# ErrorTzy/unpaper-gpu

Hardware: AMD Instinct MI355X
Metric: pages/sec + Mpixel/s, 1000-page GRAY8 A4@300dpi batch, 1/2/4/8 GPU (higher is better)
Workload: dtype u8; 1 GPU; 1000 synthetic GRAY8 A4@300dpi pages (2480x3508) per GPU, default pipeline, inputs and outputs resident in HBM; pages_per_gpu=1000, sheets_per_batch=64, streams=16, hw_queues=24, parallelism=one runner thread per device, pages sharded, no collective

## Files before the change

unpaper-gpu_amd/csrc/kernels_deskew.hip:

```cpp
#include <climits>
#include <mutex>
#include <vector>
#include <cmath>

#include "filters.h"
#include "libm_glibc.h"

namespace uph {

constexpr int kDepth = 128;
constexpr int kSliceRows = 128;
constexpr int kBandCapMax = 384;

__device__ __forceinline__ int iwave_prefix_excl(int v, int* total) {
  const int lane = threadIdx.x & 63;
  int pre = v;
  for (int o = 1; o < 64; o <<= 1) {
    int t = __shfl_up(pre, o, 64);
    if (lane >= o) pre += t;
  }
  *total = __shfl(pre, 63, 64);
  return pre - v;
}

// ... 112 lines not shown
    R.nseg[t] = 0;
    R.flag[t] = 1;
    if (act) R.list[atomicAdd(R.nlist, 1)] = t;
    return;
  }
  const LineSetup L = line_setup(masks[s], g, g.edge_shift[e][0], 0, table->slope[a]);
  const int scan = L.scan;
  int4* sg = R.segs + (int64_t)t * kLineSegs;
  int ns = 0, last = 0;
  bool over = false;
  float X = L.X;
  const float st = L.stepX;
  int i = 0;
  while (scan > 0) {
    if (ns >= kLineSegs) {
      over = true;
      break;
    }
    const float sign = X > 0.0f ? 1.0f : -1.0f;
    const double T = (double)fabsf(X), sig = (double)st * (double)sign;
    int64_t nn = 0;
    double du = 0.0;
    if (X != 0.0f) {
      int E;
      frexpf(fabsf(X), &E);
      if (E < -100) {
        over = true;
        break;
      }
      const double lo = ldexp(1.0, E - 1), hi = ldexp(1.0, E), u = ldexp(1.0, E - 24);
      const double q = ldexp(sig, 24 - E);
      const double fqd = floor(q);
      const int64_t fq = (int64_t)fqd;
      const bool tie = q - fqd == 0.5;
      if (!tie || !(((int64_t)ldexp(T, 24 - E)) & 1)) {
        const int64_t dq = tie ? (fq & 1 ? fq + 1 : fq) : (int64_t)floor(q + 0.5);
        const int64_t H = (int64_t)ldexp(hi - T, 24 - E), G = (int64_t)ldexp(T - lo, 24 - E);
        const int64_t rem = scan - 1 - i;
        auto div24 = [](int64_t c, int64_t d) -> int64_t {
          return d > c ? 0 : (int64_t)((uint32_t)c / (uint32_t)d);
        };
        if (dq > 0) {
          const int64_t c = H - fq - 1;
          nn = c >= 0 ? div24(c, dq) + 1 : 0;
        } else if (dq < 0) {
          const int64_t c = G + fq;
          nn = c >= 0 ? div24(c, -dq) + 1 : 0;
        } else {
          nn = (q >= 0.0 || G >= 1) ? rem : 0;
        }
        if (nn > rem) nn = rem;
        du = (double)dq * u;
      }
    }
    const float Ts = sign * (float)T, ds = sign * (float)du;
    sg[ns++] = make_int4(i, (int32_t)nn, __float_as_int(Ts), __float_as_int(ds));
    i += (int)nn;
    if (i >= scan - 1) {
      last = (int)fmaf((float)nn, ds, Ts);
      break;
    }
    X = sign * (float)(T + (double)nn * du) + st;
    i++;
  }
  const int first = scan > 0 ? (int)L.X : 0;
  R.ends[2 * t] = first;
  R.ends[2 * t + 1] = over ? first : last;
  const int se = t / na, lo = over ? first : imin(first, last), hi = over ? first : imax(first, last);
  atomicMin(&slo[se - se_base], lo);
  atomicMax(&shi[se - se_base], hi);
  R.nseg[t] = over ? 0 : ns;
  R.flag[t] = over;
  if (over) R.list[atomicAdd(R.nlist, 1)] = t;
  }();
  __syncthreads();
  const int tl = imin(nlines, (int)((blockIdx.x + 1) * blockDim.x)) - 1;
  const int ng = tl >= 0 ? tl / na - se_base + 1 : 0;
  if ((int)threadIdx.x < ng && slo[threadIdx.x] <= shi[threadIdx.x]) {
    atomicMin(&R.blo[se_base + threadIdx.x], slo[threadIdx.x]);
    atomicMax(&R.bhi[se_base + threadIdx.x], shi[threadIdx.x]);
  }
}

__device__ __forceinline__ bool band_range(const RotScratch& R, int tbase, int na, int sxh,
                                           int band_cap, int32_t* bx0, int32_t* bw) {
  const int se = tbase / na;
  int32_t lo = R.blo[se], hi = R.bhi[se];
  if (sxh > 0) hi += kDepth - 1;
  else lo -= kDepth - 1;
  *bx0 = lo;
  *bw = hi - lo + 1;
  return *bw <= band_cap && lo <= hi;
}

constexpr int kBandThreads = 512;
__global__ void __launch_bounds__(kBandThreads, 4)
    k_rot_band_g(PlaneRef img, RotGeom g, const RotTable* table, const Rect* masks,
                 const int32_t* mask_active, int count, int max_scan, RotScratch R, int fmt,
                 int band_cap) {
  const int sl = blockIdx.x, e = blockIdx.y, s = blockIdx.z;
  const int na = table->nangles;
  const int sxh = g.edge_shift[e][0];
  if (g.edge_shift[e][1] != 0 || (mask_active && !mask_active[s])) return;
  const Rect mask = masks[s];
  const LineSetup LS = line_setup(mask, g, sxh, 0, 0.0f);
  const int i0 = sl * kSliceRows, i1 = imin(LS.scan, i0 + kSliceRows);
  if (i0 >= i1) return;
  const int tbase = (s * g.nedges + e) * na;
  int32_t bx0, bw;
  if (!band_range(R, tbase, na, sxh, band_cap, &bx0, &bw)) return;
  extern __shared__ __attribute__((aligned(16))) uint16_t pre[];
  uint8_t* raw = reinterpret_cast<uint8_t*>(pre) + kSliceRows * bw;
  const Rect nm = normalize(mask);
  const int32_t xlo = imax(nm.x0, 0), xhi = imin(nm.x1, g.W - 1);
  const int32_t ylo = imax(nm.y0, 0), yhi = imin(nm.y1, g.H - 1);
  const int32_t ystart = (int32_t)LS.Y;
  const uint8_t* base = plane_ptr(img, s);
  const int rows = i1 - i0;
  {
    const int lane = threadIdx.x & 63, w = threadIdx.x >> 6;
    constexpr int kPer = kBandCapMax / 64;
    for (int r = w; r < rows; r += kBandThreads / 64) {
      const int32_t y = ystart + i0 + r;
      const bool rok = (y >= ylo) & (y <= yhi);
      const uint8_t* row = base + (int64_t)(rok ? y : ylo) * img.P.pitch;
      uint8_t v[kPer];
#pragma unroll
      for (int k = 0; k < kPer; k++) {
        const int c = lane + 64 * k;
        const int32_t x = bx0 + c;
        const bool ok = rok & (c < bw) & (x >= xlo) & (x <= xhi);
        const int32_t xo = ok ? x : xlo;
        uint32_t d;
        if (fmt == F_GRAY8) d = row[xo];
        else if (fmt == F_Y400A) d = row[2 * xo];
        else d = dark_of(load_px_row<F_RGB24>(row, xo));
        v[k] = (uint8_t)((255 - d) & -(int)ok);
      }
#pragma unroll
      for (int k = 0; k < kPer; k++) {
        const int c = lane + 64 * k;
        if (c < bw) raw[r * bw + c] = v[k];
      }
    }
  }
  __syncthreads();
  const int c = threadIdx.x;
  uint32_t acc = 0;
  for (int k0 = 0; k0 < kSliceRows; k0 += 32) {
    uint32_t colv[8];
    if (c < bw) {
#pragma unroll
      for (int k = 0; k < 8; k++) {
        uint32_t wv = 0;
#pragma unroll
        for (int j = 0; j < 4; j++) {
          const int r = k0 + 4 * k + j;
          wv |= (r < rows ? (uint32_t)raw[r * bw + c] : 0u) << (8 * j);
        }
        colv[k] = wv;
      }
    }
    __syncthreads();
    if (c < bw) {
#pragma unroll
      for (int k = 0; k < 8; k++) {
#pragma unroll
        for (int j = 0; j < 4; j++) {
          const int r = k0 + 4 * k + j;
          acc += (colv[k] >> (8 * j)) & 0xFFu;
          if (r < rows) pre[r * bw + c] = (uint16_t)acc;
        }
      }
    }
  }
  __syncthreads();
  const int lane = threadIdx.x & 63, w = threadIdx.x >> 6;
  constexpr int nw = kBandThreads / 64;
  const int32_t o0 = sxh * lane - bx0, o1 = sxh * (lane + 64) - bx0;
  const int ns = rot_slices(max_scan);
  for (int a = w; a < na; a += nw) {
    const int t = __builtin_amdgcn_readfirstlane(tbase + a);
    int32_t cA = 0, cB = 0;
    {
      const int nsg = __builtin_amdgcn_readfirstlane(R.nseg[t]);
      const int4 mine = lane < nsg ? R.segs[(int64_t)t * kLineSegs + lane] : make_int4(INT_MAX, 0, 0, 0);
      const int iA = i0 + lane, iB = i0 + 64 + lane;
      int q0 = 0;
      while (q0 + 1 < nsg && __builtin_amdgcn_readlane(mine.x, q0 + 1) <= i0) q0++;
      const int nxt = q0 + 1 < nsg ? __builtin_amdgcn_readlane(mine.x, q0 + 1) : INT_MAX;
      if (nxt >= i1) {
        const int b = __builtin_amdgcn_readlane(mine.x, q0);
        const float T = __int_as_float(__builtin_amdgcn_readlane(mine.z, q0));
        const float d = __int_as_float(__builtin_amdgcn_readlane(mine.w, q0));
        if (lane < rows) cA = (int)fmaf((float)(iA - b), d, T);
        if (lane + 64 < rows) cB = (int)fmaf((float)(iB - b), d, T);
      } else {
        int qA = q0, qB = q0;
        for (int q = q0 + 1; q < nsg; q++) {
          const int s0 = __builtin_amdgcn_readlane(mine.x, q);
          if (s0 >= i1) break;
          qA = iA >= s0 ? q : qA;
          qB = iB >= s0 ? q : qB;
        }
        const int bA = __shfl(mine.x, qA, 64), bB = __shfl(mine.x, qB, 64);
        const float TA = __int_as_float(__shfl(mine.z, qA, 64)), dA = __int_as_float(__shfl(mine.w, qA, 64));
        const float TB = __int_as_float(__shfl(mine.z, qB, 64)), dB = __int_as_float(__shfl(mine.w, qB, 64));
        if (lane < rows) cA = (int)fmaf((float)(iA - bA), dA, TA);
        if (lane + 64 < rows) cB = (int)fmaf((float)(iB - bB), dB, TB);
      }
    }
    const int32_t upA = __shfl_up(cA, 1, 64), upB = __shfl_up(cB, 1, 64);
    const int32_t lastA = __builtin_amdgcn_readlane(cA, 63);
    const bool stA = lane < rows && (lane == 0 || upA != cA);
    const bool stB = lane + 64 < rows && (lane == 0 ? lastA != cB : upB != cB);
    unsigned long long MA = __ballot(stA), MB = __ballot(stB);
    int acc0 = 0, acc1 = 0;
    int rs = 0;
    int32_t x = __builtin_amdgcn_readlane(cA, 0);
    MA &= MA - 1;
    for (;;) {
      int re;
      int32_t nx = 0;
      if (MA) {
        re = __ffsll((long long)MA) - 1;
        nx = __builtin_amdgcn_readlane(cA, re);
        MA &= MA - 1;
      } else if (MB) {
        const int b = __ffsll((long long)MB) - 1;
        re = 64 + b;
        nx = __builtin_amdgcn_readlane(cB, b);
        MB &= MB - 1;
      } else {
        re = rows;
      }
      const uint16_t* pe = pre + (re - 1) * bw + x;
      acc0 += pe[o0];
      acc1 += pe[o1];
      if (rs > 0) {
        const uint16_t* ps = pre + (rs - 1) * bw + x;
        acc0 -= ps[o0];
        acc1 -= ps[o1];
      }
      if (re >= rows) break;
      rs = re;
      x = nx;
    }
    uint16_t* P = R.part + ((int64_t)t * ns + sl) * kDepth;
    P[lane] = (uint16_t)acc0;
    P[lane + 64] = (uint16_t)acc1;
  }
}

__global__ void __launch_bounds__(256) k_rot_final(RotGeom g, const RotTable* table,
                                                   const Rect* masks, const int32_t* mask_active,
                                                   int mask_index, int32_t* peaks, int count,
                                                   int max_scan, RotScratch R, int band_cap) {
  const int na = table->nangles;
  const int nlines = count * g.nedges * na;
  const int t = blockIdx.x * 4 + (threadIdx.x >> 6);
  const int lane = threadIdx.x & 63;
  if (t >= nlines) return;
  const int a = t % na, e = (t / na) % g.nedges, s = t / (na * g.nedges);
  int32_t* out = peaks + (((int64_t)s * g.max_masks + mask_index) * 4 + e) * na + a;
  if (mask_active && !mask_active[s]) {
    if (lane == 0) *out = 0;
    return;
  }
  if (R.flag[t]) return;
  const int sxh = g.edge_shift[e][0];
  const LineSetup LS = line_setup(masks[s], g, sxh, 0, table->slope[a]);
  int32_t bx0, bw;
  if (LS.scan <= 0) {
    if (lane == 0) *out = 0;
    return;
  }
  if (!band_range(R, (s * g.nedges + e) * na, na, sxh, band_cap, &bx0, &bw)) {
    if (lane == 0) {
      R.flag[t] = 1;
      R.list[atomicAdd(R.nlist, 1)] = t;
    }
    return;
  }
  const int ns = rot_slices(max_scan), nsl = (LS.scan + kSliceRows - 1) / kSliceRows;
  int B[2] = {0, 0};
#pragma unroll 4
  for (int q = 0; q < nsl; q++) {
    const uint32_t v = reinterpret_cast<const uint32_t*>(R.part + ((int64_t)t * ns + q) * kDepth)[lane];
    B[0] += (int)(v & 0xFFFFu);
    B[1] += (int)(v >> 16);
  }
  const int maxAbs = (int)(255 * g.scan_size * g.scan_depth);
  const int pre1 = B[0] + B[1];
  int tot;
  const int ex = iwave_prefix_excl(pre1, &tot);
  int kfail = 2;
  for (int k = 1; k >= 0; k--) {
    const int before = ex + (k ? B[0] : 0);
    if (!(before < maxAbs && 2 * lane + k < LS.maxDepth)) kfail = k;
  }
  const unsigned long long F = __ballot(kfail < 2);
  if (!F) {
    const int up1 = __shfl_up(B[1], 1, 64);
    const int prev0 = lane == 0 ? 0 : up1;
    int md = max(B[0] - prev0, B[1] - B[0]);
    for (int o = 32; o > 0; o >>= 1) md = max(md, __shfl_xor(md, o, 64));
    const int last = __shfl(B[1], 63, 64);
    if (lane == 0) {
      R.state[4 * t] = tot;
      R.state[4 * t + 1] = last;
      R.state[4 * t + 2] = md > 0 ? md : 0;
      R.state[4 * t + 3] = 1;
      R.flag[t] = 1;
      R.list[atomicAdd(R.nlist, 1)] = t;
    }
    return;
  }
  const int fl = __ffsll((long long)F) - 1;
  const int stop = 2 * fl + __shfl(kfail, fl, 64);
  const int up = __shfl_up(B[1], 1, 64);
  int prev = lane == 0 ? 0 : up;
  int md = INT_MIN;
  for (int k = 0; k < 2; k++) {
    if (2 * lane + k < stop) md = max(md, B[k] - prev);
    prev = B[k];
  }
  for (int o = 32; o > 0; o >>= 1) md = max(md, __shfl_xor(md, o, 64));
  const int maxDiff = md > 0 ? md : 0;
  if (lane == 0) *out = stop < LS.maxDepth ? maxDiff : 0;
// ... 52 lines not shown
    const int32_t ystart = (int32_t)LS.Y;
    for (int i = threadIdx.x; i < scan; i += blockDim.x) {
      px[i] = seg_col(segs_s, nsg, i);
      py[i] = ystart + i;
    }
  } else if (threadIdx.x == 0) {
    float X = LS.X, Y = LS.Y;
    for (int i = 0; i < scan; i++) {
      px[i] = (int)X;
      py[i] = (int)Y;
      X += LS.stepX;
      Y += LS.stepY;
    }
  }
  if (threadIdx.x == 0) {
    done_flag = 0;
    result = 0;
  }
  __syncthreads();
  const int lane = threadIdx.x & 63, w = threadIdx.x >> 6;
  const uint8_t* base = plane_ptr(img, s);
  const Rect nm = normalize(mask);
  int carry_acc = 0, last = 0, maxDiff = 0;
  int dstart = 0;
  if (resume) {
    carry_acc = R.state[4 * t];
    last = R.state[4 * t + 1];
    maxDiff = R.state[4 * t + 2];
    dstart = kDepth;
  }
  for (int d0 = dstart; d0 < maxDepth; d0 += 64) {
    const int dep = d0 + lane;
    int acc = 0;
#pragma unroll 8
    for (int i = w; i < scan; i += kWaves) {
      const int32_t x = px[i] + sxh * dep, y = py[i] + syv * dep;
      const bool ok = (x >= nm.x0) & (x <= nm.x1) & (y >= nm.y0) & (y <= nm.y1) & (x >= 0) &
                      (y >= 0) & (x < g.W) & (y < g.H);
      const Px p = load_px_row<FMT>(base + (int64_t)(ok ? y : 0) * img.P.pitch, ok ? x : 0);
      acc += (255 - (int)dark_of(p)) & -(int)ok;
    }
    part[w][lane] = acc;
    __syncthreads();
    if (w == 0) {
      int B = 0;
#pragma unroll
      for (int k = 0; k < kWaves; k++) B += part[k][lane];
      int tot;
      const int before = carry_acc + iwave_prefix_excl(B, &tot);
      const bool exec = before < maxAbs && dep < maxDepth;
      const unsigned long long X_ = __ballot(!exec);
      const int stop = X_ ? __ffsll((long long)X_) - 1 : 64;
      const int up = __shfl_up(B, 1, 64);
      const int prevB = lane == 0 ? last : up;
      const int diff = B - prevB;
      int md = lane < stop ? diff : INT_MIN;
      for (int o = 32; o > 0; o >>= 1) md = max(md, __shfl_xor(md, o, 64));
      if (md > maxDiff) maxDiff = md;
      if (stop < 64) {
        if (lane == 0) {
          result = (d0 + stop) < maxDepth ? maxDiff : 0;
          done_flag = 1;
        }
      } else {
        carry_acc += tot;
        last = __shfl(B, 63, 64);
      }
    }
    __syncthreads();
    if (done_flag) break;
  }
  if (threadIdx.x == 0) *out = done_flag ? result : 0;
}

template <int FMT>
static void launch_rot_t(const PlaneRef& img, const RotGeom& g, const RotTable* table,
                         const Rect* masks, const int32_t* mask_active, int mask_index,
                         int32_t* peaks, int count, hipStream_t st, int nangles, int max_scan,
                         const RotScratch& R, float max_abs_angle) {
  const float tn = tanf(fminf(fabsf(max_abs_angle), 1.5f));
  const int band_cap =
      imin(kBandCapMax, (int)ceilf((float)imax(max_scan, 1) * tn) + kDepth + 4);
  const size_t band_lds = sizeof(uint16_t) * kSliceRows * (size_t)band_cap;
  allow_dynamic_lds((const void*)k_rot_band_g, band_lds);
  UPH_LAUNCH_DIAG(1, k_rot_band_g, dim3(rot_slices(max_scan), g.nedges, count),
                  dim3(kBandThreads), band_lds, st, img, g, table, masks, mask_active, count,
                  max_scan, R, (int)FMT, band_cap);
  const int nlines = count * g.nedges * nangles;
  UPH_LAUNCH_DIAG(128, k_rot_final, dim3((nlines + 3) / 4), dim3(256), 0, st, g, table, masks,
                  mask_active, mask_index, peaks, count, max_scan, R, band_cap);
  const size_t lds = sizeof(int32_t) * 2 * (size_t)(max_scan > 0 ? max_scan : 1);
  allow_dynamic_lds((const void*)k_rot_line<FMT>, lds);
  UPH_LAUNCH_DIAG(128, k_rot_line<FMT>, dim3(imin(nlines, 1024)), dim3(kWalkThreads), lds, st, img, g,
                  table, masks, mask_active, mask_index, peaks, count, max_scan, R);
}

void launch_rotation_peaks(const PlaneRef& img, const RotGeom& g, const RotTable* table,
                           const Rect* masks, const int32_t* mask_active, int mask_index,
                           int32_t* peaks, int count, hipStream_t st, int nangles,
                           int max_scan, int32_t* lines, float max_abs_angle) {
  if (g.nedges <= 0 || nangles <= 0) return;
  const int nlines = count * g.nedges * nangles;
  const RotScratch R = rot_scratch(lines, nlines, max_scan);
  if (hipMemsetAsync(R.nlist, 0, sizeof(int32_t), st) != hipSuccess ||
      hipMemsetAsync(R.blo, 0x7F, sizeof(int32_t) * nlines, st) != hipSuccess ||
      hipMemsetAsync(R.bhi, 0x80, sizeof(int32_t) * nlines, st) != hipSuccess)
    return;
  UPH_LAUNCH_DIAG(16, k_rot_points, dim3((nlines + 255) / 256), dim3(256), 0, st, g, table, masks,
                  mask_active, count, R);
  switch (img.P.fmt) {
    case F_GRAY8:
      launch_rot_t<F_GRAY8>(img, g, table, masks, mask_active, mask_index, peaks, count, st,
                            nangles, max_scan, R, max_abs_angle);
      break;
    case F_Y400A:
      launch_rot_t<F_Y400A>(img, g, table, masks, mask_active, mask_index, peaks, count, st,
                            nangles, max_scan, R, max_abs_angle);
      break;
    default:
      launch_rot_t<F_RGB24>(img, g, table, masks, mask_active, mask_index, peaks, count, st,
                            nangles, max_scan, R, max_abs_angle);
      break;
  }
}

}

namespace uph {

int rotation_angles(const UphipDeskewParameters& p, RotTable* t) {
  int n = 0;
  for (float r = 0.0; r <= p.deskewScanRangeRad;
       r = (r >= 0.0) ? -(r + p.deskewScanStepRad) : -r) {
    if (n >= kMaxAngles) return -1;
    t->angle[n] = r;
    t->slope[n] = tanf(r);
    n++;
  }
  t->nangles = n;
  return n;
}

float combine_edge_rotations(const float* rotation, int count, float deviation_rad) {
  float total = 0.0;
  for (int i = 0; i < count; i++) total += rotation[i];
  float average = total / count;
  total = 0.0;
  static float (*volatile pw)(float, float) = powf;
  for (int i = 0; i < count; i++) total += pw(rotation[i] - average, 2);
  float deviation = sqrtf(total);
  return deviation <= deviation_rad ? average : 0.0f;
}

const uint32_t* glibc_pow2_table(int* n) {
  static std::vector<uint32_t> table;
  static bool ok = false;
  static std::once_flag once;
  std::call_once(once, [] {
    static float (*volatile pw)(float, float) = powf;
    glibc::build_pow2_table(pw, table);
    ok = true;
    for (uint32_t v : table) ok = ok && v != 0xffffffffu;
  });
  *n = (int)table.size();
  return ok ? table.data() : nullptr;
}

}
```

unpaper-gpu_amd/csrc/filters.h:

```cpp
#pragma once

#include "scan.h"

namespace uph {

struct SheetBits {
  uint32_t* nbits = nullptr;
  uint32_t* bbits = nullptr;
  int64_t stride = 0;
  bool vsum = false;
  bool rm = false;
};

struct GrayGeom {
  int32_t W, H;
  int32_t cw, ch;
  int32_t ncx, ncy;
  int32_t tw, th;
  int32_t tsx, tsy;
  int32_t ntx, nty;
  int32_t scan_w, scan_h, step_x, step_y;
  uint8_t black_thr, abs_thr;
};
bool gray_geometry(int32_t W, int32_t H, const UphipGrayfilterParameters& p, uint8_t black_thr,
                   GrayGeom* g);
size_t gray_scratch_bytes(const GrayGeom& g);
bool launch_grayfilter(const PlaneRef& img, const GrayGeom& g, void* scratch,
                       int64_t scratch_stride, int count, hipStream_t st,
                       uint32_t* colsum = nullptr, int64_t colsum_stride = 0);
constexpr int kGrayStripMaxW = 16384;
constexpr int kGrayMaxCh = 255;
inline bool gray_cells_by_strips(const GrayGeom& g, int fmt) {
  return fmt == F_GRAY8 && g.W <= kGrayStripMaxW && g.ch <= kGrayMaxCh;
}
constexpr int kGrayRowLds = 32 * 1024;
inline size_t gray_rows_lds(const GrayGeom& g) {
  return 2 * sizeof(uint32_t) * (size_t)g.th * g.ncx;
}
inline bool gray_tiles_in_lds(const GrayGeom& g) { return gray_rows_lds(g) <= (size_t)kGrayRowLds; }

struct BlurGeom {
  int32_t W, H;
  int32_t sw, sh, step_y;
  int32_t bpr;
  int32_t T;
  int32_t nrect;
  uint8_t white;
  float intensity;
};
bool blur_geometry(int32_t W, int32_t H, const UphipBlurfilterParameters& p, uint8_t white,
                   BlurGeom* g);
size_t blur_scratch_bytes(const BlurGeom& g);
bool blur_bits_usable(const BlurGeom& g, int fmt);
enum BlurCountsArm : int32_t {
  BLUR_COUNTS_NONE,
  BLUR_COUNTS_BITS,
  BLUR_COUNTS_GRAY_V16,
  BLUR_COUNTS_GRAY,
  BLUR_COUNTS_GENERIC,
};
inline BlurCountsArm blur_counts_arm(const BlurGeom& g, int fmt, bool have_bits, bool aligned16) {
  if (have_bits) return BLUR_COUNTS_BITS;
  if (g.nrect <= 0) return BLUR_COUNTS_NONE;
  if (fmt == F_GRAY8 && g.sh <= 65535 && g.W <= (1 << 16))
    return aligned16 ? BLUR_COUNTS_GRAY_V16 : BLUR_COUNTS_GRAY;
  return BLUR_COUNTS_GENERIC;
}
constexpr int kBlurLanesMax = 120;
constexpr size_t kBlurResolveLds = 64 * 1024;
enum BlurResolveArm : int32_t {
  BLUR_RESOLVE_WAVE,
  BLUR_RESOLVE_WAVE_CHUNKED,
  BLUR_RESOLVE_GENERIC,
  BLUR_RESOLVE_GENERIC_HBM,
};
inline size_t blur_resolve_lds(const BlurGeom& g) {
  return sizeof(uint64_t) * ((size_t)g.nrect + 3 * (size_t)(g.bpr + 2));
}
inline BlurResolveArm blur_resolve_arm(const BlurGeom& g) {
  const bool scalar = g.bpr >= 1 && g.bpr + 8 <= kBlurLanesMax && (int64_t)g.sw * g.sh < (1ll << 31);
  if (scalar && g.bpr > 32 && g.bpr <= 112) return BLUR_RESOLVE_WAVE_CHUNKED;
  if (scalar) return BLUR_RESOLVE_WAVE;
  return blur_resolve_lds(g) <= kBlurResolveLds ? BLUR_RESOLVE_GENERIC : BLUR_RESOLVE_GENERIC_HBM;
}
void launch_blurfilter(const PlaneRef& img, const BlurGeom& g, void* scratch,
                       int64_t scratch_stride, int count, hipStream_t st, const SheetBits& bits);

struct NoiseGeom {
  int32_t W, H;
  int32_t intensity;
  uint8_t white;
  int32_t capacity;
  int32_t all_seq;
  int32_t diag;
  uint32_t* bbits;
  int64_t bb_stride;
};
bool noise_geometry(int32_t W, int32_t H, uint64_t intensity, uint8_t white, NoiseGeom* g);
size_t noise_scratch_bytes(const NoiseGeom& g);
void launch_noisefilter(const PlaneRef& img, const NoiseGeom& g, void* scratch,
                        int64_t scratch_stride, SheetCtl* ctl, int count, hipStream_t st,
                        const SheetBits& bits);
inline int32_t noise_bit_words(int32_t W) { return (W + 31) >> 5; }
inline int noise_group_threads(int32_t W, int32_t H) {
  return (int64_t)W * H > (16 << 20) ? 1024 : 256;
}
constexpr int kNoiseBuckets = 4096;
__host__ __device__ inline int noise_bucket_shift(int32_t H) {
  int b = 0;
  while (((H - 1) >> b) >= kNoiseBuckets) b++;
  return b;
}

struct BlackBar {
  Rect r;
  int32_t dir;
  int32_t excluded;
};
struct BlackGeom {
  int32_t W, H;
  int32_t nbars;
  int32_t nbars_h;
// ... 50 lines not shown
```

unpaper-gpu_amd/csrc/kernels_gray.hip:

```cpp
#include "filters_common.h"

namespace uph {

__host__ __device__ static inline int32_t gcd_i(int32_t a, int32_t b) {
  a = a < 0 ? -a : a;
  b = b < 0 ? -b : b;
  while (b) {
    int32_t t = a % b;
    a = b;
    b = t;
  }
  return a;
}

bool gray_geometry(int32_t W, int32_t H, const UphipGrayfilterParameters& p, uint8_t black_thr,
                   GrayGeom* g) {
  if (p.scan_size.width <= 0 || p.scan_size.height <= 0 || p.scan_step.horizontal <= 0 ||
      p.scan_step.vertical <= 0)
    return false;
  g->W = W;
  g->H = H;
  g->scan_w = p.scan_size.width;
  g->scan_h = p.scan_size.height;
  g->step_x = p.scan_step.horizontal;
// ... 71 lines not shown
  const int s = blockIdx.z;
  GrayPtrs P = gray_ptrs(g, scratch + s * sstride);
  if (blockIdx.x == 0 && threadIdx.x == 0) *P.nund = 0;
  const uint8_t* base = plane_ptr(img, s);
  const int64_t pitch = img.P.pitch;
  extern __shared__ __attribute__((aligned(16))) uint16_t cols16[];
  const int32_t wq = (g.W + 7) & ~7;
  uint16_t* cdark = cols16;
  uint16_t* clight = cols16 + wq;
  uint32_t* ctot = reinterpret_cast<uint32_t*>(cols16 + 2 * wq);
  if (colsum)
    for (int32_t x = threadIdx.x; x < g.W; x += blockDim.x) ctot[x] = 0;
  const int32_t n8 = (g.W + 7) >> 3;
  const uint32_t kadd = (256u - ((uint32_t)g.black_thr + 1u)) * 0x00010001u;
  const int32_t cy_end = imin((int32_t)(blockIdx.x + 1) * kGrayStrips, g.ncy);
  for (int32_t cy = blockIdx.x * kGrayStrips; cy < cy_end; cy++) {
    const int32_t y0 = cy * g.ch, y1 = imin(y0 + g.ch, g.H);
    for (int32_t d = threadIdx.x; d < n8; d += blockDim.x) {
      uint32_t l[4] = {0, 0, 0, 0}, ge[4] = {0, 0, 0, 0};
      auto add = [&](uint2 v) {
        const uint32_t w[4] = {v.x & 0x00FF00FFu, (v.x >> 8) & 0x00FF00FFu, v.y & 0x00FF00FFu,
                               (v.y >> 8) & 0x00FF00FFu};
#pragma unroll
        for (int j = 0; j < 4; j++) {
          l[j] += w[j];
          ge[j] += (w[j] + kadd) & 0x01000100u;
        }
      };
      const uint8_t* p = base + (int64_t)y0 * pitch + 8 * d;
      int32_t y = y0;
      for (; y + 4 <= y1; y += 4, p += 4 * pitch) {
        uint2 v[4];
#pragma unroll
        for (int k = 0; k < 4; k++) v[k] = *reinterpret_cast<const uint2*>(p + k * pitch);
#pragma unroll
        for (int k = 0; k < 4; k++) add(v[k]);
      }
      for (; y < y1; y++, p += pitch) add(*reinterpret_cast<const uint2*>(p));
      const uint32_t rows2 = (uint32_t)(y1 - y0) * 0x00010001u;
      uint32_t dk[4];
#pragma unroll
      for (int j = 0; j < 4; j++) dk[j] = rows2 - (ge[j] >> 8);
      const uint32_t sel_lo = 0x05040100u, sel_hi = 0x07060302u;
      const uint4 dv = make_uint4(__builtin_amdgcn_perm(dk[1], dk[0], sel_lo),
                                  __builtin_amdgcn_perm(dk[1], dk[0], sel_hi),
                                  __builtin_amdgcn_perm(dk[3], dk[2], sel_lo),
                                  __builtin_amdgcn_perm(dk[3], dk[2], sel_hi));
      const uint4 lv = make_uint4(__builtin_amdgcn_perm(l[1], l[0], sel_lo),
                                  __builtin_amdgcn_perm(l[1], l[0], sel_hi),
                                  __builtin_amdgcn_perm(l[3], l[2], sel_lo),
                                  __builtin_amdgcn_perm(l[3], l[2], sel_hi));
      *reinterpret_cast<uint4*>(cdark + 8 * d) = dv;
      *reinterpret_cast<uint4*>(clight + 8 * d) = lv;
    }
    __syncthreads();
    for (int32_t cx = threadIdx.x; cx < g.ncx; cx += blockDim.x) {
      const int32_t x0 = cx * g.cw, x1 = imin(x0 + g.cw, g.W);
      uint32_t dark = 0, light = 0;
      for (int32_t x = x0; x < x1; x++) {
        dark += cdark[x];
        light += clight[x];
      }
      const size_t c = (size_t)cy * g.ncx + cx;
      P.dark[c] = dark;
      P.light[c] = light;
    }
    if (colsum)
      for (int32_t x = threadIdx.x; x < g.W; x += blockDim.x) ctot[x] += clight[x];
    __syncthreads();
  }
  if (colsum) {
    uint32_t* out = colsum + (int64_t)s * colsum_stride;
    for (int32_t x = threadIdx.x; x < g.W; x += blockDim.x)
      if (ctot[x]) atomicAdd(out + x, ctot[x]);
  }
}

__device__ __forceinline__ uint32_t cell_pixels(const GrayGeom& g, int32_t cx, int32_t cy) {
  const int32_t w = imin((cx + 1) * g.cw, g.W) - cx * g.cw;
  const int32_t h = imin((cy + 1) * g.ch, g.H) - cy * g.ch;
  return (w > 0 && h > 0) ? (uint32_t)(w * h) : 0u;
}

template <class Light>
__device__ __forceinline__ uint8_t gray_tile_inv0(const GrayGeom& g, int32_t tx, int32_t ty,
                                                  Light light) {
  const Rect r = clip(rect_from_size(tx * g.step_x, ty * g.step_y, g.scan_w, g.scan_h), g.W, g.H);
  const uint64_t count = count_pixels(r);
  uint64_t sum = 0;
  const int32_t cx0 = tx * g.tsx, cy0 = ty * g.tsy;
  for (int32_t j = 0; j < g.th; j++) {
    const int32_t cy = cy0 + j;
    if (cy >= g.ncy) break;
    for (int32_t i = 0; i < g.tw; i++) {
      const int32_t cx = cx0 + i;
      if (cx >= g.ncx) break;
      sum += light(cx, cy);
    }
  }
  if (r.x1 < r.x0 || r.y1 < r.y0) sum = 0;
  return (uint8_t)(0xFFull - sum / count);
}

__device__ uint8_t gray_tile_inv(const GrayGeom& g, const GrayPtrs& P, int32_t tx, int32_t ty,
                                 int mode) {
  const Rect r = clip(rect_from_size(tx * g.step_x, ty * g.step_y, g.scan_w, g.scan_h), g.W, g.H);
  const uint64_t count = count_pixels(r);
  uint64_t sum = 0;
  const int32_t cx0 = tx * g.tsx, cy0 = ty * g.tsy;
  for (int32_t j = 0; j < g.th; j++) {
    const int32_t cy = cy0 + j;
    if (cy >= g.ncy) break;
    for (int32_t i = 0; i < g.tw; i++) {
      const int32_t cx = cx0 + i;
      if (cx >= g.ncx) break;
      const size_t c = (size_t)cy * g.ncx + cx;
      bool white = false;
      if (mode) {
        for (int32_t oy = cy - g.th + 1; oy <= cy && !white; oy++) {
          if (oy < 0 || oy % g.tsy) continue;
          const int32_t uy = oy / g.tsy;
          if (uy >= g.nty || uy > ty) continue;
          for (int32_t ox = cx - g.tw + 1; ox <= cx; ox++) {
            if (ox < 0 || ox % g.tsx) continue;
            const int32_t ux = ox / g.tsx;
            if (ux >= g.ntx) continue;
            if (uy == ty && ux >= tx) continue;
            if (P.tile[(size_t)uy * g.ntx + ux] == 2) {
              white = true;
              break;
            }
          }
        }
      }
      sum += white ? 255u * cell_pixels(g, cx, cy) : P.light[c];
    }
  }
  if (r.x1 < r.x0 || r.y1 < r.y0) sum = 0;
  return (uint8_t)(0xFFull - sum / count);
}

__device__ __forceinline__ bool gray_cell_wiped(const GrayGeom& g, const uint8_t* tile, int32_t cx,
                                                int32_t cy) {
  const int32_t uy0 = imax(0, (cy - g.th + g.tsy) / g.tsy), uy1 = imin(cy / g.tsy, g.nty - 1);
  const int32_t ux0 = imax(0, (cx - g.tw + g.tsx) / g.tsx), ux1 = imin(cx / g.tsx, g.ntx - 1);
  for (int32_t uy = uy0; uy <= uy1; uy++)
    for (int32_t ux = ux0; ux <= ux1; ux++)
      if (tile[(size_t)uy * g.ntx + ux] == 2) return true;
  return false;
}

__global__ void __launch_bounds__(256) k_gray_tiles(GrayGeom g, uint8_t* scratch, int64_t sstride) {
  const int s = blockIdx.y;
  GrayPtrs P = gray_ptrs(g, scratch + s * sstride);
  const int32_t t = blockIdx.x * 256 + threadIdx.x;
  const int32_t ntiles = g.ntx * g.nty;
  bool und = false;
  if (t < ntiles) {
    const int32_t tx = t % g.ntx, ty = t / g.ntx;
    uint32_t dark = 0;
    for (int32_t j = 0; j < g.th; j++) {
      const int32_t cy = ty * g.tsy + j;
      if (cy >= g.ncy) break;
      for (int32_t i = 0; i < g.tw; i++) {
        const int32_t cx = tx * g.tsx + i;
        if (cx >= g.ncx) break;
        dark += P.dark[(size_t)cy * g.ncx + cx];
      }
    }
    uint8_t st = 0;
    if (dark == 0) {
      st = gray_tile_inv(g, P, tx, ty, 0) < g.abs_thr ? 2 : 1;
      und = st == 1;
    }
    P.tile[t] = st;
  }
  const unsigned long long M = __ballot(und);
  if (M && (threadIdx.x & 63) == __ffsll((long long)M) - 1) atomicAdd(P.nund, (uint32_t)__popcll(M));
}

__global__ void __launch_bounds__(256) k_gray_tiles_rows(GrayGeom g, uint8_t* scratch,
                                                         int64_t sstride) {
  const int s = blockIdx.y;
  GrayPtrs P = gray_ptrs(g, scratch + s * sstride);
  const int32_t ty = blockIdx.x, cy0 = ty * g.tsy;
  const int32_t nr = imax(0, imin(g.th, g.ncy - cy0));
  extern __shared__ uint32_t gcl[];
  uint32_t* sd = gcl;
  uint32_t* sl = gcl + nr * g.ncx;
  for (int32_t i = threadIdx.x; i < nr * g.ncx; i += 256) {
    const size_t c = (size_t)cy0 * g.ncx + i;
    sd[i] = P.dark[c];
    sl[i] = P.light[c];
  }
  __syncthreads();
  bool und_any = false;
  for (int32_t tx = threadIdx.x; tx - (int32_t)threadIdx.x < g.ntx; tx += 256) {
    bool und = false;
    if (tx < g.ntx) {
      const int32_t cx0 = tx * g.tsx;
      uint32_t dark = 0;
      for (int32_t j = 0; j < nr; j++)
        for (int32_t i = 0; i < g.tw && cx0 + i < g.ncx; i++) dark += sd[j * g.ncx + cx0 + i];
      uint8_t st = 0;
      if (dark == 0) {
        const uint8_t inv = gray_tile_inv0(g, tx, ty, [&](int32_t cx, int32_t cy) {
          return sl[(cy - cy0) * g.ncx + cx];
        });
        st = inv < g.abs_thr ? 2 : 1;
        und = st == 1;
      }
      P.tile[(size_t)ty * g.ntx + tx] = st;
    }
    const unsigned long long M = __ballot(und);
    if (M && (threadIdx.x & 63) == __ffsll((long long)M) - 1) atomicAdd(P.nund, (uint32_t)__popcll(M));
    und_any |= und;
  }
  (void)und_any;
}

__global__ void __launch_bounds__(1024) k_gray_decide(GrayGeom g, uint8_t* scratch,
                                                      int64_t sstride) {
  const int s = blockIdx.x;
  GrayPtrs P = gray_ptrs(g, scratch + s * sstride);
  if (*P.nund == 0) return;
  const int32_t ntiles = g.ntx * g.nty;
  __shared__ int32_t changed;
  for (int iter = 0; iter < ntiles + 1; iter++) {
    if (threadIdx.x == 0) changed = 0;
    __syncthreads();
    for (int32_t t = threadIdx.x; t < ntiles; t += blockDim.x) {
      if (P.tile[t] != 1) continue;
      const int32_t tx = t % g.ntx, ty = t / g.ntx;
      if (gray_tile_inv(g, P, tx, ty, 1) < g.abs_thr) {
        P.tile[t] = 3;
        changed = 1;
      }
    }
    __threadfence_block();
    __syncthreads();
    if (!changed) break;
    for (int32_t t = threadIdx.x; t < ntiles; t += blockDim.x)
      if (P.tile[t] == 3) P.tile[t] = 2;
    __threadfence_block();
    __syncthreads();
  }
}

template <int FMT>
__global__ void __launch_bounds__(256) k_gray_wipe(PlaneRef img, GrayGeom g, uint8_t* scratch,
                                                   int64_t sstride, uint32_t* colsum,
                                                   int64_t colsum_stride) {
  const int s = blockIdx.z;
  const int32_t cx = blockIdx.x * 256 + threadIdx.x, cy = blockIdx.y;
  if (cx >= g.ncx) return;
  GrayPtrs P = gray_ptrs(g, scratch + s * sstride);
  if (FMT != F_Y400A && P.light[(size_t)cy * g.ncx + cx] == 255u * cell_pixels(g, cx, cy)) return;
  if (!gray_cell_wiped(g, P.tile, cx, cy)) return;
  uint8_t* base = plane_ptr(img, s);
  const int32_t x0 = cx * g.cw, x1 = imin(x0 + g.cw, g.W);
  const int32_t y0 = cy * g.ch, y1 = imin(y0 + g.ch, g.H);
  if (FMT == F_GRAY8 && colsum) {
    uint32_t* out = colsum + (int64_t)s * colsum_stride;
    for (int32_t x = x0; x < x1; x++) {
      uint32_t add = 0;
      for (int32_t y = y0; y < y1; y++) add += 255u - base[(int64_t)y * img.P.pitch + x];
      if (add) atomicAdd(out + x, add);
    }
  }
  for (int32_t y = y0; y < y1; y++) {
    uint8_t* row = base + (int64_t)y * img.P.pitch;
    for (int32_t x = x0; x < x1; x++) white_px<FMT>(row, x);
  }
}

template <int FMT>
static bool launch_gray_t(const PlaneRef& img, const GrayGeom& g, uint8_t* scr, int64_t ss,
                          int count, hipStream_t st, uint32_t* colsum, int64_t cs) {
  dim3 grid((g.ncx + 255) / 256, g.ncy, count);
  const bool strips = gray_cells_by_strips(g, FMT);
  if (!strips) colsum = nullptr;
  if (strips) {
    const size_t wq = (size_t)((g.W + 7) & ~7);
    const int n8 = (g.W + 7) >> 3;
    const int threads = imin(1024, (n8 + 63) & ~63);
    UPH_LAUNCH_DIAG(32, k_gray_cells_g, dim3((g.ncy + kGrayStrips - 1) / kGrayStrips, 1, count),
                    dim3(threads), 4 * wq + (colsum ? 4 * (size_t)g.W : 0), st, img, g, scr, ss,
                    colsum, cs);
  } else {
    hipLaunchKernelGGL(k_gray_cells<FMT>, grid, dim3(256), 0, st, img, g, scr, ss);
  }
  const int32_t ntiles = g.ntx * g.nty;
  if (gray_tiles_in_lds(g))
    hipLaunchKernelGGL(k_gray_tiles_rows, dim3(g.nty, count), dim3(256), gray_rows_lds(g), st, g, scr,
                       ss);
  else
    hipLaunchKernelGGL(k_gray_tiles, dim3((ntiles + 255) / 256, count), dim3(256), 0, st, g, scr,
                       ss);
  if (!(diag_skip() & 4))
    hipLaunchKernelGGL(k_gray_decide, dim3(count), dim3(1024), 0, st, g, scr, ss);
  hipLaunchKernelGGL(k_gray_wipe<FMT>, grid, dim3(256), 0, st, img, g, scr, ss, colsum, cs);
  return colsum != nullptr;
}

bool launch_grayfilter(const PlaneRef& img, const GrayGeom& g, void* scratch,
                       int64_t scratch_stride, int count, hipStream_t st, uint32_t* colsum,
                       int64_t colsum_stride) {
  uint8_t* scr = (uint8_t*)scratch;
  switch (img.P.fmt) {
    case F_GRAY8:
      return launch_gray_t<F_GRAY8>(img, g, scr, scratch_stride, count, st, colsum, colsum_stride);
    case F_Y400A:
      return launch_gray_t<F_Y400A>(img, g, scr, scratch_stride, count, st, nullptr, 0);
    default:
      return launch_gray_t<F_RGB24>(img, g, scr, scratch_stride, count, st, nullptr, 0);
  }
}

}
```

Baseline: 32650 pages/s.

## Restructure deskew band kernel: templated format, vectorized GRAY8 loads, prefetched segments

The rotation band kernel becomes a template on pixel format, and the block grows from 512 to 1024 threads. For GRAY8 it loads band rows as aligned 32-bit words with masked edge bytes, instead of one byte per lane with per-pixel bounds checks. Segment rows for the next angle are prefetched while the current angle is processed. Uniform parameters are pinned to scalar registers, and the prefix-sum walk is split into two branch-free loops over the ballot masks. The aim is to cut global-load instruction count, latency stalls and control overhead, at the cost of more complex edge handling and higher register and LDS pressure per block.

Result: no change. 32930 pages/s (median of 6 runs) (+0.8%).

```diff
diff --git a/unpaper-gpu_amd/csrc/kernels_deskew.hip b/unpaper-gpu_amd/csrc/kernels_deskew.hip
--- a/unpaper-gpu_amd/csrc/kernels_deskew.hip
+++ b/unpaper-gpu_amd/csrc/kernels_deskew.hip
@@ -218,65 +218,170 @@
   }
 }
 
-__device__ __forceinline__ bool band_range(const RotScratch& R, int tbase, int na, int sxh,
-                                           int band_cap, int32_t* bx0, int32_t* bw) {
-  const int se = tbase / na;
-  int32_t lo = R.blo[se], hi = R.bhi[se];
+__device__ __forceinline__ bool band_range_of(int32_t lo, int32_t hi, int sxh, int band_cap,
+                                              int32_t* bx0, int32_t* bw) {
   if (sxh > 0) hi += kDepth - 1;
   else lo -= kDepth - 1;
   *bx0 = lo;
   *bw = hi - lo + 1;
   return *bw <= band_cap && lo <= hi;
 }
-
-constexpr int kBandThreads = 512;
-__global__ void __launch_bounds__(kBandThreads, 4)
-    k_rot_band_g(PlaneRef img, RotGeom g, const RotTable* table, const Rect* masks,
-                 const int32_t* mask_active, int count, int max_scan, RotScratch R, int fmt,
-                 int band_cap) {
+__device__ __forceinline__ bool band_range(const RotScratch& R, int tbase, int na, int sxh,
+                                           int band_cap, int32_t* bx0, int32_t* bw) {
+  const int se = tbase / na;
+  return band_range_of(R.blo[se], R.bhi[se], sxh, band_cap, bx0, bw);
+}
+
+constexpr int kBandThreads = 1024;
+constexpr int kBandWaves = kBandThreads / 64;
+constexpr int kBandRowsPerWave = kSliceRows / kBandWaves;
+static_assert(kLineSegs <= 64 && (kLineSegs & (kLineSegs - 1)) == 0, "a segment row is loaded by lane & (kLineSegs-1)");
+static_assert(4 * 64 * 2 >= kBandCapMax + 3, "two dwords a lane cover a GRAY8 band row from a column rounded down to 4");
+
+struct SegRow {
+  int4 v;
+  int32_t n;
+};
+__device__ __forceinline__ SegRow seg_row_load(const RotScratch& R, int t, int lane) {
+  SegRow r;
+  int tv = t;
+  asm volatile("" : "+v"(tv));
+  r.n = R.nseg[tv];
+  r.v = R.segs[(int64_t)t * kLineSegs + (lane & (kLineSegs - 1))];
+  return r;
+}
+
+template <int FMT>
+__global__ void __launch_bounds__(kBandThreads, 8)
+    k_rot_band_g(PlaneRef img, RotGeom g, int na, const Rect* masks, const int32_t* mask_active,
+                 int max_scan, RotScratch R, int band_cap) {
   const int sl = blockIdx.x, e = blockIdx.y, s = blockIdx.z;
-  const int na = table->nangles;
-  const int sxh = g.edge_shift[e][0];
-  if (g.edge_shift[e][1] != 0 || (mask_active && !mask_active[s])) return;
+  const int se = s * g.nedges + e;
+  const int32_t* const anyp = R.blo + se;
+  const int32_t act = *(mask_active ? mask_active + s : anyp);
+  const int32_t curp = *(img.ctl ? &img.ctl[s].cur : anyp);
   const Rect mask = masks[s];
+  const int32_t blo = R.blo[se], bhi = R.bhi[se];
+  const int sxh = g.edge_shift[e][0], syv = g.edge_shift[e][1];
+  asm volatile("" ::"s"(act), "s"(curp), "s"(mask.x0), "s"(mask.y0), "s"(mask.x1), "s"(mask.y1),
+               "s"(blo), "s"(bhi), "s"(sxh), "s"(syv), "s"(g.scan_size), "s"(g.W), "s"(g.H),
+               "s"(na), "s"(band_cap), "s"(max_scan), "s"(img.which), "s"(img.P.base[0]),
+               "s"(img.P.base[1]), "s"(img.P.pitch), "s"(img.P.stride), "s"(R.segs), "s"(R.nseg),
+               "s"(R.part));
+  if (syv != 0 || (mask_active && !act)) return;
   const LineSetup LS = line_setup(mask, g, sxh, 0, 0.0f);
   const int i0 = sl * kSliceRows, i1 = imin(LS.scan, i0 + kSliceRows);
   if (i0 >= i1) return;
-  const int tbase = (s * g.nedges + e) * na;
+  const int tbase = se * na;
   int32_t bx0, bw;
-  if (!band_range(R, tbase, na, sxh, band_cap, &bx0, &bw)) return;
+  if (!band_range_of(blo, bhi, sxh, band_cap, &bx0, &bw)) return;
+  const int lane = threadIdx.x & 63, w = __builtin_amdgcn_readfirstlane(threadIdx.x >> 6);
+  SegRow ahead = seg_row_load(R, tbase + imin(w, na - 1), lane);
   extern __shared__ __attribute__((aligned(16))) uint16_t pre[];
   uint8_t* raw = reinterpret_cast<uint8_t*>(pre) + kSliceRows * bw;
   const Rect nm = normalize(mask);
   const int32_t xlo = imax(nm.x0, 0), xhi = imin(nm.x1, g.W - 1);
   const int32_t ylo = imax(nm.y0, 0), yhi = imin(nm.y1, g.H - 1);
   const int32_t ystart = (int32_t)LS.Y;
-  const uint8_t* base = plane_ptr(img, s);
+  int pk = img.which;
+  if (img.ctl) pk = img.which ? 1 - curp : curp;
+  const uint8_t* base = (pk ? img.P.base[1] : img.P.base[0]) + (int64_t)s * img.P.stride;
   const int rows = i1 - i0;
-  {
-    const int lane = threadIdx.x & 63, w = threadIdx.x >> 6;
+  if (FMT == F_GRAY8) {
+    const int32_t bxa = bx0 & ~3;
+    const int sh = bx0 - bxa;
+    const int32_t cl = imax(xlo - bx0, 0), ch = imin(xhi - bx0, bw - 1);
+    const int32_t xmax = (int32_t)img.P.pitch - 4;
+    const int cf = (4 - sh) & 3;
+    const int ct = cf + ((bw - cf) & ~3);
+    constexpr int kEdgeIters = kSliceRows * 8 / kBandThreads;
+    static_assert(kEdgeIters * kBandThreads == kSliceRows * 8, "edge slots divide among the threads");
+    uint8_t ev[kEdgeIters];
+#pragma unroll
+    for (int i = 0; i < kEdgeIters; i++) {
+      const int idx = threadIdx.x + i * kBandThreads, r = idx >> 3, q = idx & 7;
+      const int c = q < 4 ? q : ct + q - 4;
+      const int32_t y = ystart + i0 + r, x = bx0 + c;
+      ev[i] = base[(int64_t)imin(imax(y, 0), g.H - 1) * img.P.pitch + imin(imax(x, 0), g.W - 1)];
+    }
+    int c0[2];
+    uint32_t okm[2];
+    bool full[2];
+#pragma unroll
+    for (int k = 0; k < 2; k++) {
+      c0[k] = 4 * (lane + 64 * k) - sh;
+      okm[k] = 0;
+#pragma unroll
+      for (int q = 0; q < 4; q++) {
+        const int c = c0[k] + q;
+        okm[k] |= ((c >= cl) & (c <= ch)) ? 0xFFu << (8 * q) : 0u;
+      }
+      full[k] = (c0[k] >= 0) & (c0[k] + 3 < bw);
+    }
+    uint32_t v[kBandRowsPerWave][2];
+#pragma unroll
+    for (int j = 0; j < kBandRowsPerWave; j++) {
+      const int32_t y = ystart + i0 + w + kBandWaves * j;
+      const uint8_t* row = base + (int64_t)imin(imax(y, 0), g.H - 1) * img.P.pitch;
+#pragma unroll
+      for (int k = 0; k < 2; k++) {
+        const int32_t xg = bxa + 4 * (lane + 64 * k);
+        v[j][k] = *reinterpret_cast<const uint32_t*>(row + imin(imax(xg, 0), xmax));
+      }
+    }
+#pragma unroll
+    for (int i = 0; i < kEdgeIters; i++) {
+      const int idx = threadIdx.x + i * kBandThreads, r = idx >> 3, q = idx & 7;
+      const int c = q < 4 ? q : ct + q - 4;
+      const int32_t y = ystart + i0 + r;
+      const bool ok = (y >= ylo) & (y <= yhi) & (c >= cl) & (c <= ch);
+      if ((r < rows) & (q < 4 ? q < cf : ((q < 7) & (c < bw))))
+        raw[r * bw + c] = (uint8_t)((255 - (uint32_t)ev[i]) & -(int)ok);
+    }
+#pragma unroll
+    for (int j = 0; j < kBandRowsPerWave; j++) {
+      const int r = w + kBandWaves * j;
+      const int32_t y = ystart + i0 + r;
+      const uint32_t rowm = ((y >= ylo) & (y <= yhi)) ? ~0u : 0u;
+      if (r < rows) {
+#pragma unroll
+        for (int k = 0; k < 2; k++) {
+          const uint32_t val = ~v[j][k] & okm[k] & rowm;
+          if (full[k]) __builtin_memcpy(raw + r * bw + c0[k], &val, 4);
+        }
+      }
+    }
+  } else {
     constexpr int kPer = kBandCapMax / 64;
-    for (int r = w; r < rows; r += kBandThreads / 64) {
-      const int32_t y = ystart + i0 + r;
-      const bool rok = (y >= ylo) & (y <= yhi);
-      const uint8_t* row = base + (int64_t)(rok ? y : ylo) * img.P.pitch;
-      uint8_t v[kPer];
-#pragma unroll
-      for (int k = 0; k < kPer; k++) {
-        const int c = lane + 64 * k;
-        const int32_t x = bx0 + c;
-        const bool ok = rok & (c < bw) & (x >= xlo) & (x <= xhi);
-        const int32_t xo = ok ? x : xlo;
-        uint32_t d;
-        if (fmt == F_GRAY8) d = row[xo];
-        else if (fmt == F_Y400A) d = row[2 * xo];
-        else d = dark_of(load_px_row<F_RGB24>(row, xo));
-        v[k] = (uint8_t)((255 - d) & -(int)ok);
-      }
-#pragma unroll
-      for (int k = 0; k < kPer; k++) {
-        const int c = lane + 64 * k;
-        if (c < bw) raw[r * bw + c] = v[k];
+    constexpr int kGroup = FMT == F_RGB24 ? 2 : 4;
+    static_assert(kBandRowsPerWave % kGroup == 0, "whole groups");
+    for (int j0 = 0; j0 < kBandRowsPerWave; j0 += kGroup) {
+      uint8_t v[kGroup][kPer];
+#pragma unroll
+      for (int j = 0; j < kGroup; j++) {
+        const int32_t y = ystart + i0 + w + kBandWaves * (j0 + j);
+        const bool rok = (y >= ylo) & (y <= yhi);
+        const uint8_t* row = base + (int64_t)imin(imax(y, 0), g.H - 1) * img.P.pitch;
+#pragma unroll
+        for (int k = 0; k < kPer; k++) {
+          const int c = lane + 64 * k;
+          const int32_t x = bx0 + c;
+          const bool ok = rok & (c < bw) & (x >= xlo) & (x <= xhi);
+          const int32_t xo = imin(imax(x, 0), g.W - 1);
+          const uint32_t d = dark_of(load_px_row<FMT>(row, xo));
+          v[j][k] = (uint8_t)((255 - d) & -(int)ok);
+        }
+      }
+#pragma unroll
+      for (int j = 0; j < kGroup; j++) {
+        const int r = w + kBandWaves * (j0 + j);
+        if (r < rows) {
+#pragma unroll
+          for (int k = 0; k < kPer; k++) {
+            const int c = lane + 64 * k;
+            if (c < bw) raw[r * bw + c] = v[j][k];
+          }
+        }
       }
     }
   }
@@ -292,7 +397,8 @@
 #pragma unroll
         for (int j = 0; j < 4; j++) {
           const int r = k0 + 4 * k + j;
-          wv |= (r < rows ? (uint32_t)raw[r * bw + c] : 0u) << (8 * j);
+          const uint32_t b = raw[r * bw + c];
+          wv |= (r < rows ? b : 0u) << (8 * j);
         }
         colv[k] = wv;
       }
@@ -311,16 +417,16 @@
     }
   }
   __syncthreads();
-  const int lane = threadIdx.x & 63, w = threadIdx.x >> 6;
-  constexpr int nw = kBandThreads / 64;
   const int32_t o0 = sxh * lane - bx0, o1 = sxh * (lane + 64) - bx0;
   const int ns = rot_slices(max_scan);
-  for (int a = w; a < na; a += nw) {
-    const int t = __builtin_amdgcn_readfirstlane(tbase + a);
+  for (int a = w; a < na; a += kBandWaves) {
+    const int t = tbase + a;
+    const SegRow cur = ahead;
+    ahead = seg_row_load(R, tbase + imin(a + kBandWaves, na - 1), lane);
     int32_t cA = 0, cB = 0;
     {
-      const int nsg = __builtin_amdgcn_readfirstlane(R.nseg[t]);
-      const int4 mine = lane < nsg ? R.segs[(int64_t)t * kLineSegs + lane] : make_int4(INT_MAX, 0, 0, 0);
+      const int nsg = __builtin_amdgcn_readfirstlane(cur.n);
+      const int4 mine = lane < nsg ? cur.v : make_int4(INT_MAX, 0, 0, 0);
       const int iA = i0 + lane, iB = i0 + 64 + lane;
       int q0 = 0;
       while (q0 + 1 < nsg && __builtin_amdgcn_readlane(mine.x, q0 + 1) <= i0) q0++;
@@ -352,35 +458,32 @@
     const bool stB = lane + 64 < rows && (lane == 0 ? lastA != cB : upB != cB);
     unsigned long long MA = __ballot(stA), MB = __ballot(stB);
     int acc0 = 0, acc1 = 0;
-    int rs = 0;
     int32_t x = __builtin_amdgcn_readlane(cA, 0);
     MA &= MA - 1;
-    for (;;) {
-      int re;
-      int32_t nx = 0;
-      if (MA) {
-        re = __ffsll((long long)MA) - 1;
-        nx = __builtin_amdgcn_readlane(cA, re);
-        MA &= MA - 1;
-      } else if (MB) {
-        const int b = __ffsll((long long)MB) - 1;
-        re = 64 + b;
-        nx = __builtin_amdgcn_readlane(cB, b);
-        MB &= MB - 1;
-      } else {
-        re = rows;
-      }
-      const uint16_t* pe = pre + (re - 1) * bw + x;
-      acc0 += pe[o0];
-      acc1 += pe[o1];
-      if (rs > 0) {
-        const uint16_t* ps = pre + (rs - 1) * bw + x;
-        acc0 -= ps[o0];
-        acc1 -= ps[o1];
-      }
-      if (re >= rows) break;
-      rs = re;
+    while (MA) {
+      const int re = __ffsll((long long)MA) - 1;
+      MA &= MA - 1;
+      const int32_t nx = __builtin_amdgcn_readlane(cA, re);
+      const uint16_t* pr = pre + (re - 1) * bw;
+      const int a0 = pr[x + o0], a1 = pr[x + o1], b0 = pr[nx + o0], b1 = pr[nx + o1];
+      acc0 += a0 - b0;
+      acc1 += a1 - b1;
       x = nx;
+    }
+    while (MB) {
+      const int b = __ffsll((long long)MB) - 1;
+      MB &= MB - 1;
+      const int32_t nx = __builtin_amdgcn_readlane(cB, b);
+      const uint16_t* pr = pre + (63 + b) * bw;
+      const int a0 = pr[x + o0], a1 = pr[x + o1], b0 = pr[nx + o0], b1 = pr[nx + o1];
+      acc0 += a0 - b0;
+      acc1 += a1 - b1;
+      x = nx;
+    }
+    {
+      const uint16_t* pr = pre + (rows - 1) * bw;
+      acc0 += pr[x + o0];
+      acc1 += pr[x + o1];
     }
     uint16_t* P = R.part + ((int64_t)t * ns + sl) * kDepth;
     P[lane] = (uint16_t)acc0;
@@ -599,10 +702,10 @@
   const int band_cap =
       imin(kBandCapMax, (int)ceilf((float)imax(max_scan, 1) * tn) + kDepth + 4);
   const size_t band_lds = sizeof(uint16_t) * kSliceRows * (size_t)band_cap;
-  allow_dynamic_lds((const void*)k_rot_band_g, band_lds);
-  UPH_LAUNCH_DIAG(1, k_rot_band_g, dim3(rot_slices(max_scan), g.nedges, count),
-                  dim3(kBandThreads), band_lds, st, img, g, table, masks, mask_active, count,
-                  max_scan, R, (int)FMT, band_cap);
+  allow_dynamic_lds((const void*)k_rot_band_g<FMT>, band_lds);
+  UPH_LAUNCH_DIAG(1, k_rot_band_g<FMT>, dim3(rot_slices(max_scan), g.nedges, count),
+                  dim3(kBandThreads), band_lds, st, img, g, nangles, masks, mask_active, max_scan, R,
+                  band_cap);
   const int nlines = count * g.nedges * nangles;
   UPH_LAUNCH_DIAG(128, k_rot_final, dim3((nlines + 3) / 4), dim3(256), 0, st, g, table, masks,
                   mask_active, mask_index, peaks, count, max_scan, R, band_cap);
```

## Precompute column sums in gray tiles and wave-cooperatively wipe gray cells

Applied to the files above, without the earlier changes.

The tile kernel now builds per-column dark and light totals across the tile rows in LDS, so each tile sums a single row of column totals instead of rescanning a 2D window. This takes more dynamic LDS and an extra barrier. The wipe kernel now uses a wave ballot so groups of lanes share each wiped cell, spreading the cell's columns across lanes with coalesced row access and an unrolled column-sum loop, where before one thread walked the whole cell serially. This adds ballot and indexing overhead, and cells with width not a power of two leave some lanes idle.

New measurement: 32660 pages/s before, 32670 pages/s after (median of 2 runs). Within noise of the previous version (+0.0%).

```diff
diff --git a/unpaper-gpu_amd/csrc/filters.h b/unpaper-gpu_amd/csrc/filters.h
--- a/unpaper-gpu_amd/csrc/filters.h
+++ b/unpaper-gpu_amd/csrc/filters.h
@@ -38,6 +38,10 @@
   return 2 * sizeof(uint32_t) * (size_t)g.th * g.ncx;
 }
 inline bool gray_tiles_in_lds(const GrayGeom& g) { return gray_rows_lds(g) <= (size_t)kGrayRowLds; }
+inline size_t gray_tiles_lds_bytes(const GrayGeom& g) {
+  return ((gray_rows_lds(g) + sizeof(uint32_t) * (size_t)g.ncx + 7) & ~(size_t)7) +
+         sizeof(uint64_t) * (size_t)g.ncx;
+}
 
 struct BlurGeom {
   int32_t W, H;
diff --git a/unpaper-gpu_amd/csrc/kernels_gray.hip b/unpaper-gpu_amd/csrc/kernels_gray.hip
--- a/unpaper-gpu_amd/csrc/kernels_gray.hip
+++ b/unpaper-gpu_amd/csrc/kernels_gray.hip
@@ -177,22 +177,10 @@
   return (w > 0 && h > 0) ? (uint32_t)(w * h) : 0u;
 }
 
-template <class Light>
 __device__ __forceinline__ uint8_t gray_tile_inv0(const GrayGeom& g, int32_t tx, int32_t ty,
-                                                  Light light) {
+                                                  uint64_t sum) {
   const Rect r = clip(rect_from_size(tx * g.step_x, ty * g.step_y, g.scan_w, g.scan_h), g.W, g.H);
   const uint64_t count = count_pixels(r);
-  uint64_t sum = 0;
-  const int32_t cx0 = tx * g.tsx, cy0 = ty * g.tsy;
-  for (int32_t j = 0; j < g.th; j++) {
-    const int32_t cy = cy0 + j;
-    if (cy >= g.ncy) break;
-    for (int32_t i = 0; i < g.tw; i++) {
-      const int32_t cx = cx0 + i;
-      if (cx >= g.ncx) break;
-      sum += light(cx, cy);
-    }
-  }
   if (r.x1 < r.x0 || r.y1 < r.y0) sum = 0;
   return (uint8_t)(0xFFull - sum / count);
 }
@@ -280,29 +268,40 @@
   GrayPtrs P = gray_ptrs(g, scratch + s * sstride);
   const int32_t ty = blockIdx.x, cy0 = ty * g.tsy;
   const int32_t nr = imax(0, imin(g.th, g.ncy - cy0));
-  extern __shared__ uint32_t gcl[];
+  extern __shared__ __attribute__((aligned(16))) uint32_t gcl[];
   uint32_t* sd = gcl;
   uint32_t* sl = gcl + nr * g.ncx;
+  uint32_t* cd = gcl + 2 * g.th * g.ncx;
+  uint64_t* cl = reinterpret_cast<uint64_t*>(gcl + ((2 * g.th * g.ncx + g.ncx + 1) & ~1));
   for (int32_t i = threadIdx.x; i < nr * g.ncx; i += 256) {
     const size_t c = (size_t)cy0 * g.ncx + i;
     sd[i] = P.dark[c];
     sl[i] = P.light[c];
+  }
+  __syncthreads();
+  for (int32_t cx = threadIdx.x; cx < g.ncx; cx += 256) {
+    uint32_t d = 0;
+    uint64_t l = 0;
+    for (int32_t j = 0; j < nr; j++) {
+      d += sd[j * g.ncx + cx];
+      l += sl[j * g.ncx + cx];
+    }
+    cd[cx] = d;
+    cl[cx] = l;
   }
   __syncthreads();
   bool und_any = false;
   for (int32_t tx = threadIdx.x; tx - (int32_t)threadIdx.x < g.ntx; tx += 256) {
     bool und = false;
     if (tx < g.ntx) {
-      const int32_t cx0 = tx * g.tsx;
+      const int32_t cx0 = tx * g.tsx, cx1 = imin(cx0 + g.tw, g.ncx);
       uint32_t dark = 0;
-      for (int32_t j = 0; j < nr; j++)
-        for (int32_t i = 0; i < g.tw && cx0 + i < g.ncx; i++) dark += sd[j * g.ncx + cx0 + i];
+      for (int32_t cx = cx0; cx < cx1; cx++) dark += cd[cx];
       uint8_t st = 0;
       if (dark == 0) {
-        const uint8_t inv = gray_tile_inv0(g, tx, ty, [&](int32_t cx, int32_t cy) {
-          return sl[(cy - cy0) * g.ncx + cx];
-        });
-        st = inv < g.abs_thr ? 2 : 1;
+        uint64_t sum = 0;
+        for (int32_t cx = cx0; cx < cx1; cx++) sum += cl[cx];
+        st = gray_tile_inv0(g, tx, ty, sum) < g.abs_thr ? 2 : 1;
         und = st == 1;
       }
       P.tile[(size_t)ty * g.ntx + tx] = st;
@@ -348,24 +347,41 @@
                                                    int64_t colsum_stride) {
   const int s = blockIdx.z;
   const int32_t cx = blockIdx.x * 256 + threadIdx.x, cy = blockIdx.y;
-  if (cx >= g.ncx) return;
-  GrayPtrs P = gray_ptrs(g, scratch + s * sstride);
-  if (FMT != F_Y400A && P.light[(size_t)cy * g.ncx + cx] == 255u * cell_pixels(g, cx, cy)) return;
-  if (!gray_cell_wiped(g, P.tile, cx, cy)) return;
+  GrayPtrs P = gray_ptrs(g, scratch + s * sstride);
+  bool wipe = cx < g.ncx;
+  if (wipe && FMT != F_Y400A) wipe = P.light[(size_t)cy * g.ncx + cx] != 255u * cell_pixels(g, cx, cy);
+  if (wipe) wipe = gray_cell_wiped(g, P.tile, cx, cy);
+  const uint64_t M = __ballot(wipe);
+  if (!M) return;
+  int G = 1;
+  while (G < g.cw && G < 64) G <<= 1;
+  const int K = 64 / G, lane = threadIdx.x & 63;
+  const int grp = lane / G, c0 = lane & (G - 1);
   uint8_t* base = plane_ptr(img, s);
-  const int32_t x0 = cx * g.cw, x1 = imin(x0 + g.cw, g.W);
+  const int64_t pitch = img.P.pitch;
   const int32_t y0 = cy * g.ch, y1 = imin(y0 + g.ch, g.H);
-  if (FMT == F_GRAY8 && colsum) {
-    uint32_t* out = colsum + (int64_t)s * colsum_stride;
-    for (int32_t x = x0; x < x1; x++) {
-      uint32_t add = 0;
-      for (int32_t y = y0; y < y1; y++) add += 255u - base[(int64_t)y * img.P.pitch + x];
-      if (add) atomicAdd(out + x, add);
-    }
-  }
-  for (int32_t y = y0; y < y1; y++) {
-    uint8_t* row = base + (int64_t)y * img.P.pitch;
-    for (int32_t x = x0; x < x1; x++) white_px<FMT>(row, x);
+  uint32_t* out = FMT == F_GRAY8 && colsum ? colsum + (int64_t)s * colsum_stride : nullptr;
+  for (int k = 0; k < G; k++) {
+    if (!((M >> (k * K + grp)) & 1ull)) continue;
+    const int32_t wx = cx - lane + k * K + grp;
+    const int32_t x0 = wx * g.cw, x1 = imin(x0 + g.cw, g.W);
+    for (int32_t x = x0 + c0; x < x1; x += G) {
+      if (out) {
+        uint32_t add = 0;
+        const uint8_t* p = base + (int64_t)y0 * pitch + x;
+        int32_t y = y0;
+        for (; y + 4 <= y1; y += 4, p += 4 * pitch) {
+          uint32_t v[4];
+#pragma unroll
+          for (int j = 0; j < 4; j++) v[j] = p[j * pitch];
+#pragma unroll
+          for (int j = 0; j < 4; j++) add += 255u - v[j];
+        }
+        for (; y < y1; y++, p += pitch) add += 255u - *p;
+        if (add) atomicAdd(out + x, add);
+      }
+      for (int32_t y = y0; y < y1; y++) white_px<FMT>(base + (int64_t)y * pitch, x);
+    }
   }
 }
 
@@ -386,10 +402,11 @@
     hipLaunchKernelGGL(k_gray_cells<FMT>, grid, dim3(256), 0, st, img, g, scr, ss);
   }
   const int32_t ntiles = g.ntx * g.nty;
-  if (gray_tiles_in_lds(g))
-    hipLaunchKernelGGL(k_gray_tiles_rows, dim3(g.nty, count), dim3(256), gray_rows_lds(g), st, g, scr,
-                       ss);
-  else
+  if (gray_tiles_in_lds(g)) {
+    allow_dynamic_lds((const void*)k_gray_tiles_rows, gray_tiles_lds_bytes(g));
+    hipLaunchKernelGGL(k_gray_tiles_rows, dim3(g.nty, count), dim3(256), gray_tiles_lds_bytes(g), st, g,
+                       scr, ss);
+  } else
     hipLaunchKernelGGL(k_gray_tiles, dim3((ntiles + 255) / 256, count), dim3(256), 0, st, g, scr,
                        ss);
   if (!(diag_skip() & 4))
```
